# nncarlson/nka

Hardware: AMD Instinct MI355X
Metric: NKA updates/sec + achieved HBM GB/s at n=1e8, m=20 fp64; 1/2/4/8 GPUs (higher is better)
Workload: dtype f64

## Files before the change

### include/nka_hip_diag.h

```cpp
#ifndef NKA_HIP_DIAG_H
#define NKA_HIP_DIAG_H

#include "nka_hip_ext.h"
#include "nka_hip_vec.h"

#ifdef __cplusplus
extern "C" {
#endif

int nka_hip_set_tuning(nka_hip_t a, const char *key, int32_t value);

int nka_hip_get_skip_state(nka_hip_t a, int32_t out4[4]);

int nka_hip_set_grid(nka_hip_t a, int32_t pa_blocks_per_cu, int32_t pb_blocks_per_cu);

int nka_hip_debug_time_pa(nka_hip_t a, const double *f_dev, int32_t reps, float *ms_mean);

int nka_hip_debug_chain_sum(nka_hip_t a, const double *x_dev, const double *y_dev, int64_t n, double start, int32_t walk,
                            double *sum, float *ms);

int nka_hip_get_stamps(nka_hip_t a, double *out16);

int nka_hip_vec_set_tuning(nka_hip_vec_ws_t ws, const char *key, int32_t value);

#ifdef __cplusplus
}
#endif
// ... 2 lines not shown
```

### nka_amd/_lib.py

```python
from __future__ import annotations

import ctypes as C
import os
import subprocess

HERE = os.path.dirname(os.path.abspath(__file__))
_LIB = None

_i32p = C.POINTER(C.c_int32)
_dp = C.POINTER(C.c_double)
ALLREDUCE_FN = C.CFUNCTYPE(C.c_int, C.c_void_p, C.c_void_p, C.c_int32, C.c_void_p)
HOST_DOT_FN = C.CFUNCTYPE(C.c_double, C.c_void_p, C.c_int64, C.POINTER(C.c_double), C.POINTER(C.c_double))
HOST_ALLREDUCE_FN = C.CFUNCTYPE(C.c_int, C.c_void_p, C.POINTER(C.c_double), C.c_int32)

SIGNATURES = {
    "nka_hip_create": (C.c_int, [C.POINTER(C.c_void_p), C.c_int64, C.c_int32, C.c_double, C.c_int32, C.c_int32, C.c_void_p]),
    "nka_hip_destroy": (C.c_int, [C.c_void_p]),
    "nka_hip_clone": (C.c_int, [C.c_void_p, C.POINTER(C.c_void_p)]),
    "nka_hip_capture_safe": (C.c_int, [C.c_void_p]),
    "nka_hip_list_bound": (C.c_int, [C.c_void_p]),
    "nka_hip_set_stream": (C.c_int, [C.c_void_p, C.c_void_p]),
    "nka_hip_accel_update": (C.c_int, [C.c_void_p, C.c_void_p]),
    "nka_hip_accel_update_host": (C.c_int, [C.c_void_p, C.c_void_p]),
    "nka_hip_accel_update_swap": (C.c_int, [C.c_void_p, C.POINTER(C.c_void_p), C.POINTER(C.c_void_p)]),
# ... 144 lines not shown
    "nka_hip_batch_get_reductions": (C.c_int, [C.c_void_p, C.c_int32, _dp]),
    "nka_hip_batch_get_w": (C.c_int, [C.c_void_p, C.c_int32, C.c_int32, _dp]),
    "nka_hip_batch_get_v": (C.c_int, [C.c_void_p, C.c_int32, C.c_int32, _dp]),
    "nka_hip_batch_state_digest": (C.c_int, [C.c_void_p, C.c_int32, C.POINTER(C.c_uint64)]),
}


DIAG_SIGNATURES = {
    "nka_hip_set_tuning": (C.c_int, [C.c_void_p, C.c_char_p, C.c_int32]),
    "nka_hip_set_grid": (C.c_int, [C.c_void_p, C.c_int32, C.c_int32]),
    "nka_hip_debug_time_pa": (C.c_int, [C.c_void_p, C.c_void_p, C.c_int32, C.POINTER(C.c_float)]),
    "nka_hip_debug_chain_sum": (C.c_int, [C.c_void_p, C.c_void_p, C.c_void_p, C.c_int64, C.c_double, C.c_int32,
                                          C.POINTER(C.c_double), C.POINTER(C.c_float)]),
    "nka_hip_get_stamps": (C.c_int, [C.c_void_p, _dp]),
    "nka_hip_get_skip_state": (C.c_int, [C.c_void_p, C.POINTER(C.c_int32)]),
    "nka_hip_vec_set_tuning": (C.c_int, [C.c_void_p, C.c_char_p, C.c_int32]),
}
_DIAG = None


def diag_lib_path() -> str:
    return os.environ.get("NKA_HIP_DIAG_LIB") or os.path.join(HERE, "libnka_hip_diag.so")


def load_diag() -> C.CDLL:
    global _DIAG
    if _DIAG is None:
        path = diag_lib_path()
        if not os.path.exists(path):
            raise RuntimeError(f"{path} not found: `make -C nka_amd/csrc diag` (or __graft_entry__.build())")
# ... 54 lines not shown
```

### nka_amd/csrc/handles.hpp

```cpp
#pragma once

#include "../../include/nka_hip.h"
#include "../../include/nka_hip_ext.h"
#include "../../include/nka_hip_vec.h"
#include "nka_ctl.hpp"
#include "host_logic.hpp"
#include "rccl_dl.hpp"

#include <hip/hip_runtime.h>

#include <cstdint>
#include <string>
#include <vector>

namespace nka_detail {
int set_error(int code, const std::string &msg);
std::string last_error();
bool &span_check_failed();
int check_device_span(const void *p, int64_t n, const char *what);
int check_device_span_i32(const void *p, int64_t n, const char *what);
void invalidate_span_cache();
void register_allocation(const void *p, size_t bytes, const void *owner);
void unregister_owner(const void *owner);
void unregister_allocation(const void *p);
// ... 52 lines not shown
  int bpc[2] = {0, 0};
  char devname[64] = {0};
  int pa_pipe = -1;
  int pb_pipe = -1;
  int pb_flags = 0;
  int pb_tile = -1;
  int pb_tickets = -1;
  double *chain_pred = nullptr;
  void *chain_summ = nullptr;
  long long chain_cap = 0;
  int chain_many = -1;
  int chain_walk = 0;
  int fail_after_solve = 0;
  int prime_pad = -1;
  int skip_last = -1;
  int pa_skip = 0;
  bool state_in_global = false;
  bool serial_solve = false;
  int sum_order = NKA_HIP_SUMS_AUTO;
  bool debug = false;
  nka_hip_allreduce_fn allreduce = nullptr;
  void *allreduce_ctx = nullptr;
  ncclComm_t comm = nullptr;
  nka::P2P p2p{};
  void *p2p_mail = nullptr;
  std::vector<void *> p2p_opened;
  void *p2p_dev = nullptr;
  int p2p_ranks = 0;
  bool p2p_fused = false;
  int pa_normed = 0;
// ... 33 lines not shown
```

### nka_amd/csrc/lab.hip

```cpp
#include "handles.hpp"
#include "nka_chain.hpp"
#include "../../include/nka_hip_diag.h"

#include <algorithm>
#include <string>

using namespace nka;
using namespace nka_detail;

extern "C" {

int nka_hip_get_stamps(nka_hip_t a, double *out16) {
  if (!a || !out16) return fail(NKA_HIP_EINVAL, "null argument");
  HIP_TRY(hipSetDevice(a->device));
  HIP_TRY(hipMemcpyAsync(out16, a->ctl.stamps(), sizeof(double) * kStamps, hipMemcpyDeviceToHost, a->stream));
  HIP_TRY(hipStreamSynchronize(a->stream));
  return 0;
}

int nka_hip_get_skip_state(nka_hip_t a, int32_t out4[4]) {
  if (!a || !out4) return fail(NKA_HIP_EINVAL, "null argument");
  HIP_TRY(hipSetDevice(a->device));
  HIP_TRY(hipMemcpyAsync(out4, a->ctl.ic + IC_PLAN_SKIP, sizeof(int32_t) * 4, hipMemcpyDeviceToHost, a->stream));
  HIP_TRY(hipStreamSynchronize(a->stream));
  return 0;
}

int nka_hip_set_grid(nka_hip_t a, int32_t pa, int32_t pb) {
  if (!a) return fail(NKA_HIP_EINVAL, "null handle");
  const int32_t v[2] = {pa, pb};
  for (int i = 0; i < 2; i++) {
    if (v[i] < 0 || v[i] * a->num_cu > kMaxGrid) return fail(NKA_HIP_EINVAL, "blocks per CU out of range");
    a->bpc[i] = v[i];
  }
  return 0;
}

int nka_hip_debug_chain_sum(nka_hip_t a, const double *x, const double *y, int64_t n, double start, int32_t walk, double *sum,
                            float *ms) {
// ... 71 lines not shown
  } else if (k == "pb_tile") {
    if (value != -1 && value != 1 && value != 2) return fail(NKA_HIP_EINVAL, "pb_tile: -1 (auto), 1, 2");
    a->pb_tile = value;
  } else if (k == "pb_tickets") {
    if (value != -1 && value != 0 && value != 1 && value != 2 && value != 4 && value != 8)
      return fail(NKA_HIP_EINVAL, "pb_tickets: -1 (auto), 0 (static tile mapping), 1, 2, 4, 8 (ticket counters)");
    a->pb_tickets = value;
  } else if (k == "fail_after_solve") {
    a->fail_after_solve = value != 0;
  } else if (k == "prime_pad") {
    if (value < -1 || value > 1) return fail(NKA_HIP_EINVAL, "prime_pad: -1, 0, 1");
    a->prime_pad = value;
  } else if (k == "skip_last") {
    if (value < -1 || value > 1) return fail(NKA_HIP_EINVAL, "skip_last: -1, 0, 1");
    a->skip_last = value;
  } else if (k == "chain_many") {
    if (value < -1 || value > 1) return fail(NKA_HIP_EINVAL, "chain_many: -1, 0, 1");
    a->chain_many = value;
  } else if (k == "chain_walk") {
    a->chain_walk = value != 0;
  } else if (k == "serial_solve") {
    a->serial_solve = value != 0;
  } else if (k == "list_word") {
    a->word_off = value == 0;
  } else {
    return fail(NKA_HIP_EINVAL, "unknown tuning key: " + k);
  }
  return 0;
}

// ... 13 lines not shown
```

### nka_amd/csrc/nka_ctl.hpp

```cpp
#pragma once

#include <cstddef>
#include <cstdint>

#if defined(__HIPCC__)
#include <hip/hip_runtime.h>
#define NKA_HOST_DEVICE __host__ __device__
#else
#define NKA_HOST_DEVICE
#endif

namespace nka {

enum {
  IC_SUBSPACE = 0,
  IC_PENDING = 1,
  IC_FIRST = 2,
  IC_LAST = 3,
  IC_FREE = 4,
  IC_NEW = 5,
  IC_NCOMB = 6,
  IC_PLAN_PENDING = 7,
  IC_PLAN_FIRST = 8,
  IC_PLAN_NOLDER = 9,
// ... 1 lines not shown
  IC_NORMED = 11,
  IC_PLAN_SKIP = 12,
  IC_SKIP_HOLD = 13,
  IC_REDO = 14,
  IC_NREDO = 15,
  IC_HEADER = 16
};
enum { DC_VTOL = 0, DC_S = 1, DC_HEADER = 2 };
enum {
  PC_FIRST_W = 0,
  PC_NEW_W = 1,
  PC_NEW_V = 2,
  PC_OLD_W = 3,
  PC_OLD_V = 4,
  PC_WGT = 5,
  PC_HEADER = 8
};

constexpr int kMaxPerPass = 32;
constexpr int kMaxGrid = 4096;

constexpr int kStamps = 16;

struct Ctl {
  int32_t *ic;
  double *dc;
  int32_t mvec;
  unsigned long long *hw;
  unsigned long long seq;
  long long *pc;
  NKA_HOST_DEVICE long long *plan_w() const { return pc + PC_HEADER; }
  NKA_HOST_DEVICE long long *comb_w() const { return plan_w() + m1p(); }
  NKA_HOST_DEVICE long long *comb_v() const { return comb_w() + m1p(); }
  NKA_HOST_DEVICE long long *wtab() const { return comb_v() + m1p(); }
  NKA_HOST_DEVICE long long *vtab() const { return wtab() + (m1() + 1); }
  NKA_HOST_DEVICE constexpr int pc_count() const { return PC_HEADER + 3 * m1p() + 2 * (m1() + 1); }
  NKA_HOST_DEVICE constexpr int m1() const { return mvec + 1; }
  NKA_HOST_DEVICE constexpr int m1p() const { return mvec + 1 + kMaxPerPass; }
  NKA_HOST_DEVICE int32_t *next() const { return ic + IC_HEADER; }
  NKA_HOST_DEVICE int32_t *prev() const { return next() + (m1() + 1); }
  NKA_HOST_DEVICE int32_t *plan_slots() const { return prev() + (m1() + 1); }
  NKA_HOST_DEVICE int32_t *comb_slots() const { return plan_slots() + m1p(); }
  NKA_HOST_DEVICE constexpr int ic_count() const { return IC_HEADER + 2 * (m1() + 1) + 2 * m1p(); }
  NKA_HOST_DEVICE double *h() const { return dc + DC_HEADER; }
  NKA_HOST_DEVICE double *c() const { return h() + (m1() + 1) * (m1() + 1); }
  NKA_HOST_DEVICE double *comb_c() const { return c() + (m1() + 1); }
  NKA_HOST_DEVICE double *red() const { return comb_c() + m1p(); }
  NKA_HOST_DEVICE constexpr int red_count() const { return 2 + 2 * mvec; }
  NKA_HOST_DEVICE double *stamps() const { return red() + red_count(); }
  NKA_HOST_DEVICE constexpr int dc_count() const {
    return DC_HEADER + (m1() + 1) * (m1() + 1) + (m1() + 1) + m1p() + red_count() + kStamps;
// ... 24 lines not shown
```

### nka_amd/csrc/nka_hip.hip

```cpp
#include "handles.hpp"
#include "nka_kernels.hpp"

#include <dlfcn.h>

#include <algorithm>
#include <atomic>
#include <chrono>
#include <cmath>
#include <cstdio>
#include <cstdlib>
#include <cstring>
#include <map>
#include <mutex>
#include <set>
#include <string>
#include <vector>

using namespace nka;

namespace {
thread_local std::string g_err;
}

namespace nka_detail {
// ... 237 lines not shown
  if constexpr (COMB == 2) {
    if (maxk <= 4) return launch_combine_1<4, VEC, COMB>(a, f, pass, last);
    return launch_combine_1<32, VEC, COMB>(a, f, pass, last);
  }
#define CASE(K) \
  case K: return launch_combine_1<K, VEC, COMB>(a, f, pass, last);
  switch (maxk) {
    CASE(4) CASE(8) CASE(12) CASE(16) CASE(20) CASE(24) CASE(28) CASE(32)
  }
#undef CASE
  return 0;
}

template <int MAXK, int COMB, int W, int T = 1>
int launch_combine_win_1(const nka_hip_state *a, double *f, int bpc, int base) {
  static const int occ = occupancy_of(k_combine_win<MAXK, COMB, W, T>);
  const int64_t ntile = a->n / (kBlock * 2 * T);
  const int g = persistent_grid(a->num_cu, std::min(occ, std::max(1, bpc)), ntile);
  constexpr int words = ((COMB == 2 ? MAXK + 2 : 2 * MAXK + 1) + 5) * T;
  const int ng = nka_host::ticket_counters(a->pb_tickets, a->tickets != nullptr, ntile, T, g, words);
  const int tail = (ntile * (kBlock * 2 * T) < a->n) ? 1 : 0;
  hipLaunchKernelGGL((k_combine_win<MAXK, COMB, W, T>), dim3(g + tail), dim3(kBlock), 0, a->stream, a->ctl, a->vs, f,
                     ng > 0 ? a->tickets : nullptr, std::max(ng, 1), a->pb_flags, base);
  return g;
}

bool pb_tickets_apply(const nka_hip_state *a) {
  return nka_host::tickets_expected(a->pb_tickets, a->tickets != nullptr, a->n / (kBlock * 2), a->num_cu);
}

// ... 277 lines not shown
  hipFree(a->tickets);
  hipFree(a->ctl.pc);
  for (void *p : a->extra_allocs) hipFree(p);
  if (a->list_word) hipHostFree(a->list_word);
  hipFree(a->f_stage);
  hipFree(a->hd_scratch);
  hipFree(a->wgt);
  hipFree(a->wgt_chk);
  for (auto &e : a->ev)
    if (e) hipEventDestroy(e);
  a->ev.clear();
  delete a;
  return 0;
}

static int fetch_tables(nka_hip_t a, std::vector<long long> &pc, Ctl &t) {
  pc.assign((size_t)a->ctl.pc_count(), 0);
  HIP_TRY(hipMemcpyAsync(pc.data(), a->ctl.pc, sizeof(long long) * pc.size(), hipMemcpyDeviceToHost, a->stream));
  HIP_TRY(hipStreamSynchronize(a->stream));
  t = a->ctl;
  t.pc = pc.data();
  return 0;
}
static const double *slot_buffer(nka_hip_t a, const Ctl *tables, bool v, int slot) {
  if (tables) return buffer_at(a, v ? tables->vtab()[slot] : tables->wtab()[slot]);
  return (v ? a->vs.v : a->vs.w) + (size_t)(slot - 1) * a->vs.stride;
}
static __global__ void k_plan_pointers_from_slots(Ctl ctl) {
  if (threadIdx.x != 0 || blockIdx.x != 0) return;
  const int n = ctl.ic[IC_PLAN_NOLDER];
  for (int j = 0; j < n; j++) ctl.plan_w()[j] = ctl.wtab()[ctl.plan_slots()[j]];
  ctl.pc[PC_FIRST_W] = ctl.wtab()[ctl.ic[IC_PLAN_FIRST]];
}

int nka_hip_clone(nka_hip_t src, nka_hip_t *out) {
  if (!src || !out) return fail(NKA_HIP_EINVAL, "nka_hip_clone: null argument");
  *out = nullptr;
  nka_hip_t b = nullptr;
  if (int rc = nka_hip_create(&b, src->n, src->mvec, src->vtol, src->flavor, src->device, (void *)src->stream)) return rc;
  if (b->vs.stride != src->vs.stride || b->ctl.ic_count() != src->ctl.ic_count() || b->ctl.dc_count() != src->ctl.dc_count()) {
    nka_hip_destroy(b);
    return fail(NKA_HIP_ESTATE, "nka_hip_clone: storage geometry differs");
  }
  const size_t slot_bytes = (size_t)src->vs.stride * sizeof(double) * (size_t)(src->mvec + 1);
  hipStream_t s = src->stream;
  hipError_t e = hipSuccess;
  if (!src->swapped) {
    e = hipMemcpyAsync(b->vs.v, src->vs.v, slot_bytes, hipMemcpyDeviceToDevice, s);
    if (e == hipSuccess) e = hipMemcpyAsync(b->vs.w, src->vs.w, slot_bytes, hipMemcpyDeviceToDevice, s);
  } else {
    std::vector<long long> pc;
    Ctl t{};
// ... 16 lines not shown
  }
  if (e != hipSuccess) {
    nka_hip_destroy(b);
    return fail(NKA_HIP_EHIP, std::string("nka_hip_clone: ") + hipGetErrorString(e));
  }
  b->pending = src->pending;
  b->list_ub = src->list_ub;
  b->bpc[0] = src->bpc[0];
  b->bpc[1] = src->bpc[1];
  b->pa_pipe = src->pa_pipe;
  b->pb_pipe = src->pb_pipe;
  b->pb_tile = src->pb_tile;
  b->pb_tickets = src->pb_tickets;
  b->prime_pad = src->prime_pad;
  b->skip_last = src->skip_last;
  b->chain_walk = src->chain_walk;
  b->chain_many = src->chain_many;
  b->chain_pred = nullptr; b->chain_summ = nullptr; b->chain_cap = 0;
  b->serial_solve = src->serial_solve;
  b->sum_order = src->sum_order;
  b->shard_rank = src->shard_rank;
  b->shard_n = src->shard_n;
  b->debug = src->debug;
  if (src->allreduce != rccl_allreduce && src->allreduce != p2p_allreduce) {
    b->allreduce = src->allreduce;
    b->allreduce_ctx = src->allreduce_ctx;
    b->needs_comm = src->needs_comm;
  } else {
    b->needs_comm = true;
  }
// ... 8 lines not shown
    if (e != hipSuccess) {
      (void)hipGetLastError();
      nka_hip_destroy(b);
      return fail(e == hipErrorOutOfMemory ? NKA_HIP_ENOMEM : NKA_HIP_EHIP, std::string("nka_hip_clone: ") + hipGetErrorString(e));
    }
  }
  b->weighted = src->weighted;
  *out = b;
  return 0;
}

int nka_hip_restart(nka_hip_t a) {
  if (!a) return fail(NKA_HIP_EINVAL, "null handle");
  if (a->poisoned) return fail(NKA_HIP_ESTATE, "restart: an earlier update failed after its scalar step had been enqueued: destroy the handle");
  HIP_TRY(hipSetDevice(a->device));
  hipLaunchKernelGGL(k_restart, dim3(1), dim3(kSolveThreads), a->state_in_global ? 0 : lst_smem_bytes(a->mvec), a->stream,
                     a->ctl, a->state_in_global ? 1 : 0);
  HIP_TRY(hipGetLastError());
  a->pending = false;
  a->list_ub = 0;
  a->word_valid_after = a->seq;
  a->relaxed_after.clear();
  return 0;
}

int nka_hip_relax(nka_hip_t a) {
  if (!a) return fail(NKA_HIP_EINVAL, "null handle");
  if (a->poisoned) return fail(NKA_HIP_ESTATE, "relax: an earlier update failed after its scalar step had been enqueued: destroy the handle");
  HIP_TRY(hipSetDevice(a->device));
  hipLaunchKernelGGL(k_relax, dim3(1), dim3(kSolveThreads), a->state_in_global ? 0 : lst_smem_bytes(a->mvec), a->stream,
                     a->ctl, a->state_in_global ? 1 : 0);
  HIP_TRY(hipGetLastError());
  if (a->pending) {
    a->pending = false;
    a->list_ub = std::max(a->list_ub - 1, 0);
    if (!a->word_off && a->list_word) a->relaxed_after.push_back(a->seq);
    if (a->relaxed_after.size() > 4096) a->relaxed_after.erase(a->relaxed_after.begin(), a->relaxed_after.begin() + 2048);
  }
  return 0;
}

int nka_hip_set_vec_tol(nka_hip_t a, double vtol) {
  if (!a) return fail(NKA_HIP_EINVAL, "null handle");
  if (!(vtol > 0.0)) return fail(NKA_HIP_EINVAL, "set_vec_tol: vtol must be > 0");
// ... 2 lines not shown
  HIP_TRY(hipMemcpyAsync(a->ctl.dc + DC_VTOL, &a->vtol, sizeof(double), hipMemcpyHostToDevice, a->stream));
  HIP_TRY(hipStreamSynchronize(a->stream));
  return 0;
}

static int enqueue_solve(nka_hip_t a, int mode, long long swap_w = kNoBuffer, long long swap_v = kNoBuffer, bool gather = false,
                         int skip = 0) {
  hipStream_t s = a->stream;
  const P2P x = gather ? a->p2p : P2P{};
  if (a->mvec + 1 <= kSolveWaveMax && !a->serial_solve) {
    const size_t sm = solve_wave_smem_bytes(a->mvec);
    const int nl = a->mvec + 1;
    const long long id_stride = (a->swapped || a->captured) ? 0 : (long long)a->vs.stride, id_vbase = buffer_offset(a, a->vs.v);
#define ROWS(NL) \
  hipLaunchKernelGGL((k_solve_rows<NL>), dim3(1), dim3(kSolveThreads), sm, s, a->ctl, mode, swap_w, swap_v, id_stride, id_vbase, x, \
                     skip)
    if (nl <= 6) ROWS(6);
    else if (nl <= 11) ROWS(11);
    else if (nl <= 21) ROWS(21);
    else if (nl <= 33) ROWS(33);
    else if (nl <= 48) ROWS(48);
    else {
      if (!a->solve63_raised) {
        const hipError_t raised = hipFuncSetAttribute(reinterpret_cast<const void *>(k_solve_rows<63>),
                                                      hipFuncAttributeMaxDynamicSharedMemorySize,
                                                      (int)solve_wave_smem_bytes(kSolveWaveMax - 1));
        if (raised != hipSuccess) return fail(NKA_HIP_EHIP, std::string("raising the dynamic LDS limit failed: ") + hipGetErrorString(raised));
        a->solve63_raised = true;
      }
      ROWS(63);
    }
// ... 403 lines not shown
}

static int update_impl(nka_hip_t a, double *f, long long swap_w, long long swap_v);
static int p2p_status_after_sync(nka_hip_t a);

constexpr double kSkipLastMinBytes = 4.8e7;
static bool skip_last_applies(const nka_hip_state *a, SumsStage stage, int vec, int older_ub) {
  if (a->skip_last == 0) return false;
  if (stage != SumsStage::Rounded && stage != SumsStage::Blocked) return false;
  if (a->allreduce || a->host_dot || a->serial_solve) return false;
  if (a->mvec < 2 || a->mvec > kMaxPerPass || vec != 2 || older_ub != a->mvec) return false;
  if (a->pa_pipe != -1 && a->pa_pipe != 201) return false;
  return a->skip_last > 0 || 8.0 * (double)a->n >= kSkipLastMinBytes;
}

int nka_hip_accel_update(nka_hip_t a, double *f) { return update_impl(a, f, kNoBuffer, kNoBuffer); }

static int update_impl(nka_hip_t a, double *f, long long swap_w, long long swap_v) {
  if (!a) return fail(NKA_HIP_EINVAL, "null handle");
  if (!f && a->n > 0) return fail(NKA_HIP_EINVAL, "accel_update: f is NULL");
  HIP_TRY(hipSetDevice(a->device));
  if (int rc = nka_detail::check_device_span(f, a->n, "accel_update: f")) return rc;
  if (swap_w == kNoBuffer && f && f == a->last_acc)
    return fail(NKA_HIP_EINVAL, "accel_update: that buffer is the accelerated f lent by the previous out-of-place update (read only: "
                                "it is the stored v of the pending pair); copy it, or go on with nka_hip_accel_update_swap");
  if (a->poisoned)
    return fail(NKA_HIP_ESTATE, "accel_update: an earlier update of this handle failed after its scalar step had been enqueued "
                                "(a HIP error): the lists on the device are ahead of the stored vectors.  Destroy the handle");
  if (a->swapped && f && held_by_library(a, f))
    return fail(NKA_HIP_EINVAL, "accel_update: that buffer is held by the library (a stored vector, or a buffer handed over to "
// ... 19 lines not shown
    if (!a->captured || user_hook || a->host_dot) {
      hipStreamCaptureStatus cs = hipStreamCaptureStatusNone;
      if (hipStreamIsCapturing(s, &cs) != hipSuccess) (void)hipGetLastError();
      else if (cs != hipStreamCaptureStatusNone) {
        if (user_hook || a->host_dot)
          return fail(NKA_HIP_EINVAL, "accel_update: cannot be captured into a graph with a caller's all-reduce hook or dot product "
                                      "installed (host callbacks: a replay would not call them); the built-in RCCL hook and the "
                                      "peer-to-peer exchange can be captured");
        a->captured = a->word_off = true;
      }
    }
  }
  if (int rc = record(a, 0)) return rc;
  a->list_ub = list_bound_now(a);
  const int older_ub = a->pending ? std::max(a->list_ub - 1, 0) : a->list_ub;

  SumsResult sums{};
  const SumsStage stage = pick_sums_stage(a);
  const bool skip = skip_last_applies(a, stage, vec, older_ub);
  a->pa_skip = skip ? kSkipMay : 0;
  switch (stage) {
    case SumsStage::HostDot:        sums = sums_host_dot(a, f, mode); break;
    case SumsStage::ReferenceChain: sums = sums_reference_chain(a, f, mode, older_ub); break;
    case SumsStage::ReferenceOrder: sums = sums_reference_order(a, f, mode, older_ub); break;
    case SumsStage::Rounded:        sums = sums_rounded(a, f, vec, mode, older_ub); break;
    case SumsStage::Blocked:        sums = sums_blocked(a, f, vec, older_ub); break;
  }
  a->pa_skip = 0;
  if (sums.rc) return sums.rc;
  mode |= sums.mode_bits;
// ... 10 lines not shown
  } poison{a};
  if (a->fail_after_solve) {
    a->fail_after_solve = 0;
    return fail(NKA_HIP_EHIP, "accel_update: injected failure behind the scalar step (lab switch fail_after_solve)");
  }
  if (skip) {
    a->pa_skip = kSkipRepair;
    a->pa_normed = stage == SumsStage::Rounded ? ((mode & kSolveRcp) ? 3 : 1) : 0;
    launch_dots_win(1, a, f, 1, a->mvec - 1, 1, a->mvec);
    a->pa_skip = a->pa_normed = 0;
    HIP_TRY(hipGetLastError());
    if (int rc = enqueue_solve(a, mode, swap_w, swap_v, false, kSkipRepair)) return rc;
  }
  if (int rc = record(a, 2)) return rc;

  const int comb_ub = a->pending ? std::min(a->list_ub, (int)a->mvec) : a->list_ub;
  a->ctl.seq = (unsigned long long)(a->seq + 1);
  {
    Ctl &c = a->ctl;
    unsigned long long *const hw = c.hw;
    if (a->word_off) c.hw = nullptr;
    a->pb_flags = (swap_w != kNoBuffer ? (kPbNoStoreW | kPbNoStoreF) : 0);
    const int rc = enqueue_pb(a, f, vec, comb_ub);
    a->pb_flags = 0;
    c.hw = hw;
    if (rc) return rc;
  }
  a->seq++;
  if (int rc = record(a, 3)) return rc;

  if (a->timing_this) a->timing_count++;
  a->list_ub = comb_ub + 1;
  a->pending = true;
  if (swap_w == kNoBuffer) a->last_acc = nullptr;
  poison.armed = false;
  return 0;
}

int nka_hip_accel_update_host(nka_hip_t a, double *f_host) {
  if (!a) return fail(NKA_HIP_EINVAL, "null handle");
  if (!f_host && a->n > 0) return fail(NKA_HIP_EINVAL, "accel_update_host: f is NULL");
  HIP_TRY(hipSetDevice(a->device));
// ... 47 lines not shown
    }
  }
  return 0;
}

int nka_hip_accel_update_swap(nka_hip_t a, double **f_io, const double **f_acc) {
  if (!a) return fail(NKA_HIP_EINVAL, "null handle");
  if (!f_io || !f_acc || (!*f_io && a->n > 0)) return fail(NKA_HIP_EINVAL, "accel_update_swap: null argument");
  if (a->host_dot) return fail(NKA_HIP_ESTATE, "accel_update_swap: not with a user dot product on host copies (nka_hip_set_host_dot)");
  if (reinterpret_cast<uintptr_t>(*f_io) % 16 != 0) return fail(NKA_HIP_EINVAL, "accel_update_swap: the buffer must be 16-byte aligned");
  HIP_TRY(hipSetDevice(a->device));
  hipStreamCaptureStatus cs = hipStreamCaptureStatusNone;
  if (hipStreamIsCapturing(a->stream, &cs) != hipSuccess) (void)hipGetLastError();
  else if (cs != hipStreamCaptureStatusNone)
    return fail(NKA_HIP_ESTATE, "accel_update_swap: cannot be captured into a graph (the host chooses buffers per call)");
  if (int rc = collect_spares(a)) return rc;
  double *const in = *f_io, *const give_w = a->spare_w, *const vnew = a->spare_v;
  if (in && (in == give_w || in == vnew)) return fail(NKA_HIP_EINVAL, "accel_update_swap: that buffer is the library's own spare");
  if (in && in == a->last_acc)
    return fail(NKA_HIP_EINVAL, "accel_update_swap: that buffer is the accelerated f lent by the previous update (read only: it "
                                "is the stored v of the pending pair)");
  if (in && held_by_library(a, in))
    return fail(NKA_HIP_EINVAL, "accel_update_swap: that buffer is already held by the library (a stored vector, or a buffer "
                                "handed over earlier): two slots would share it");
  a->swapped = true;
  if (int rc = update_impl(a, in, buffer_offset(a, in), buffer_offset(a, vnew))) return rc;
  if (in) {
    a->book.lent.erase(in);
    const int64_t block = a->vs.stride * (int64_t)(a->mvec + 1);
    const bool inside = (in >= a->vs.w && in < a->vs.w + block) || (in >= a->vs.v && in < a->vs.v + block);
// ... 97 lines not shown
    if (last != k) return 0;
  }
  for (int k = fr; k != 0; k = next[k]) {
    if (tag[k]) return 0;
    tag[k] = 1;
  }
  for (int k = 1; k <= n; k++)
    if (!tag[k]) return 0;
  return 1;
}

static int get_slot(nka_hip_t a, bool v, int32_t slot, double *host_out) {
  if (!a) return fail(NKA_HIP_EINVAL, "null handle");
  if (slot < 1 || slot > a->mvec + 1) return fail(NKA_HIP_EINVAL, "slot out of range");
  HIP_TRY(hipSetDevice(a->device));
  std::vector<long long> pc;
  Ctl t{};
  if (a->swapped)
    if (int rc = fetch_tables(a, pc, t)) return rc;
  HIP_TRY(hipMemcpyAsync(host_out, slot_buffer(a, a->swapped ? &t : nullptr, v, slot), sizeof(double) * (size_t)a->n,
                         hipMemcpyDeviceToHost, a->stream));
  HIP_TRY(hipStreamSynchronize(a->stream));
  return 0;
}
int nka_hip_get_w(nka_hip_t a, int32_t slot, double *host_out) { return get_slot(a, false, slot, host_out); }
int nka_hip_get_v(nka_hip_t a, int32_t slot, double *host_out) { return get_slot(a, true, slot, host_out); }


int nka_hip_set_allreduce(nka_hip_t a, nka_hip_allreduce_fn fn, void *ctx) {
  if (!a) return fail(NKA_HIP_EINVAL, "null handle");
// ... 382 lines not shown
```

### nka_amd/csrc/nka_kernels.hpp

```cpp
#pragma once

#include "nka_chain.hpp"

namespace nka {


__global__ __launch_bounds__(128) void k_p2p_allreduce(P2P x, double *buf, int count) {
  const unsigned long long seq = *x.xseq;
  for (int i = threadIdx.x; i < count * x.n; i += blockDim.x) p2p_send_one(x, i % x.n, seq, i / x.n, buf[i / x.n]);
  __syncthreads();
  p2p_gather_block(x, buf, count);
}

template <int MAXL, int VEC, bool WGT = false>
__global__ __launch_bounds__(kBlock) void k_dots(Ctl ctl, Vecs vs, const double *__restrict__ f,
                                                 double *__restrict__ partials, int pass, int normed) {
  const double *wgt = WGT ? vs.w + ctl.pc[PC_WGT] : nullptr;
  using V = typename VecT<VEC>::type;
  constexpr int NACC = 2 * MAXL + 2;
  const int G = gridDim.x;
  const double s_n = normed ? sqrt(ctl.red()[0]) : 1.0, rs_n = 1.0 / s_n;
  const int pending = ctl.ic[IC_PLAN_PENDING];
  const int nolder = ctl.ic[IC_PLAN_NOLDER];
  const int base = pass * MAXL;
// ... 572 lines not shown
    chain_load_block(cs, regs, e0, lane, false);
    chain_store_block(cs, regs, blk_lds, lane);
    a = chain_block_serial(a, blk_lds, (int)(cs.n - e0));
  }
  if (lane == 0) red[cs.dst] = a;
#ifdef NKA_CHAIN_STAMPS
  if (lane == 0 && set == kChainProbe) {
    for (int i = 0; i < 8; i++) ctl.stamps()[8 + i] = (double)cnt[i];
    ctl.stamps()[3] = (double)tw;
  }
#endif
#undef NKA_APPLY_COUNT
}

enum { kPbNoStoreW = 1, kPbNoStoreF = 2,
       kPbNotFirst = 8, kPbNotLast = 16 };

template <int MAXK, int VEC, int COMB>
__global__ __launch_bounds__(kBlock) void k_combine(Ctl ctl, Vecs vs, double *f, int pass, int last_pass, int flags) {
  using V = typename VecT<VEC>::type;
  constexpr bool RCP = (COMB == 1);
  constexpr bool COMPACT = (COMB == 2);
  constexpr int NW = COMPACT ? 1 : MAXK;
  const int G = gridDim.x;
  const int ncomb = ctl.ic[IC_NCOMB];
  double *wnew = vs.w + ctl.pc[PC_NEW_W], *vnew = vs.w + ctl.pc[PC_NEW_V];
  const long long *cw = ctl.comb_w(), *cv = ctl.comb_v();
  const double *cc = ctl.comb_c();
  const int base = pass * MAXK;
  const bool oop = (flags & kPbNoStoreF) != 0;
  const double *src = (oop && pass > 0) ? vnew : f;
// ... 68 lines not shown
            v = RCP ? rs * v : v / s;
            if (COMPACT) v = v - w;
            wk[0][i] = w;
            vk[0][i] = v;
          }
          x = COMPACT ? x + ck[j] * v : comb1<COMB>(x, ck[j], w, v);
        }
      }
      if (store_w) wnew[i] = fin;
      if (store_v) vnew[i] = x;
      if (store_f) f[i] = x;
    }
  }
}

template <int MAXK, int COMB, int W, int T = 1>
__global__ __launch_bounds__(kBlock) void k_combine_win(Ctl ctl, Vecs vs, double *f, unsigned *tickets, int ng, int flags,
                                                        int base) {
  constexpr int VEC = 2;
  using V = typename VecT<VEC>::type;
  constexpr bool RCP = (COMB == 1);
  constexpr bool COMPACT = (COMB == 2);
  constexpr int TILE = kBlock * VEC * T;
  static_assert(MAXK % W == 0, "the ring must divide the pairs of a tile");
  NKA_STAMP0(ctl, 14);
  __shared__ unsigned s_next[2];
  const int64_t ntile = vs.n / TILE;
  const bool has_tail = ntile * TILE < vs.n;
  const int G = (int)gridDim.x - (has_tail ? 1 : 0);
  const bool tail_block = has_tail && (int)blockIdx.x == G;
  const int ncomb_all = ctl.ic[IC_NCOMB];
  const int ncomb = ncomb_all - base;
  double *wnew = vs.w + ctl.pc[PC_NEW_W], *vnew = vs.w + ctl.pc[PC_NEW_V];
  const long long *cw = ctl.comb_w() + base, *cv = ctl.comb_v() + base;
  const double *cc = ctl.comb_c() + base;
  const bool first_pass = !(flags & kPbNotFirst), last_pass = !(flags & kPbNotLast);
  const bool store_w = !(flags & kPbNoStoreW) && first_pass, store_f = !(flags & kPbNoStoreF), store_v = last_pass;
  const bool norm0 = first_pass && ctl.ic[IC_NORMED] != 0;
  const double s = ctl.dc[DC_S];
  const double rs = 1.0 / s;

  double *wk[MAXK], *vk[MAXK];
  double ck[MAXK];
  long long slw[MAXK], slv[MAXK];
#pragma unroll
  for (int j = 0; j < MAXK; j++) {
    if (!COMPACT || j == 0) slw[j] = cw[j];
    slv[j] = cv[j];
    ck[j] = cc[j];
  }
#pragma unroll
  for (int j = 0; j < MAXK; j++) {
    const bool live = j < ncomb;
// ... 210 lines not shown

constexpr int kSolveWaveMax = 63;

__host__ __device__ inline size_t solve_wave_smem_bytes(int mvec) {
  const int nl = mvec + 1;
  size_t b = (lst_smem_bytes(mvec) + 15) / 16 * 16;
  b += (size_t)((nl + 1) * (nl + 1) + 3 * nl + (2 + 2 * mvec)) * sizeof(double);
  b += (size_t)(3 * nl + 1) * sizeof(int32_t);
  b = (b + 7) / 8 * 8;
  b += (size_t)(2 * (nl + 1)) * sizeof(long long);
  return b;
}

template <int NLMAX>
__global__ __launch_bounds__(kSolveThreads) void k_solve_rows(Ctl ctl, int mode, long long swap_w, long long swap_v,
                                                              long long id_stride, long long id_vbase, P2P x, int skip) {
  extern __shared__ __attribute__((aligned(16))) unsigned char smem[];
  const int lane = threadIdx.x;
  if (skip_repair_idle(ctl, skip)) return;
  if (x.base != nullptr) p2p_gather_block(x, ctl.red(), ctl.red_count());
  const int m1 = ctl.m1(), NL = m1, LDA = NL + 1, M = ctl.mvec, nh = (m1 + 1) * (m1 + 1);
  Lst L;
  L.m1 = m1;
  L.mvec = M;
  L.h = reinterpret_cast<double *>(smem);
  L.c = L.h + nh;
  L.next = reinterpret_cast<int32_t *>(L.c + (m1 + 1));
  L.prev = L.next + (m1 + 1);
  double *A = reinterpret_cast<double *>(smem + (lst_smem_bytes(ctl.mvec) + 15) / 16 * 16);
  double *bb = A + (NL + 1) * LDA + 2 * NL;
  double *redL = bb + NL;
  int32_t *ord = reinterpret_cast<int32_t *>(redL + (2 + 2 * M));
  int32_t *psL = ord + 2 * NL;
  long long *wtL = reinterpret_cast<long long *>((reinterpret_cast<uintptr_t>(psL + NL + 1) + 7) / 8 * 8);
// ... 201 lines not shown
      }
    }
    NKA_STAMP(ctl, 7);
    nk = __builtin_popcountll(alive & listmask);
    if (lane < nl && ((alive >> lane) & 1)) {
      const int r = __builtin_popcountll(alive & ((1ull << lane) - 1));
      ctl.comb_slots()[r] = myord;
      ctl.comb_c()[r] = yr;
      ctl.plan_slots()[r] = myord;
      const long long wb = wtL[myord];
      ctl.comb_w()[r] = wb;
      ctl.comb_v()[r] = vtL[myord];
      ctl.plan_w()[r] = wb;
      L.c[myord] = yr;
    }
  } else if (L.subspace) {
    for (int k = L.first; k != 0; k = L.next[k]) ord[nk++] = k;
    __syncthreads();
    for (int p = lane; p < nk; p += kSolveThreads) bb[p] = L.c[ord[p]];
    for (int idx = lane; idx < nk * nk; idx += kSolveThreads) {
      const int p = idx / nk, q = idx - p * nk;
      if (p >= q) A[p * LDA + q] = L.H(ord[p], ord[q]);
    }
    __syncthreads();
    for (int i = 0; i < nk; i++) {
      const double ci = bb[i] / A[i * LDA + i];
      __syncthreads();
      if (lane == 0) bb[i] = ci;
      for (int j = i + 1 + lane; j < nk; j += kSolveThreads) bb[j] = bb[j] - A[j * LDA + i] * ci;
      __syncthreads();
// ... 25 lines not shown
    if (entry_first != 0 && !normed && entry_pending) ctl.ic[IC_NRELAX] += 1;
    ctl.ic[IC_NEW] = slot;
    ctl.ic[IC_NCOMB] = nk;
    ctl.ic[IC_NORMED] = normed;
    lst_store_scalars(L, ctl);
    ctl.ic[IC_PLAN_PENDING] = L.pending;
    ctl.ic[IC_PLAN_FIRST] = L.first;
    ctl.ic[IC_PLAN_NOLDER] = nk;
    int hold = hold_in > 0 ? hold_in - 1 : 0;
    if (skip & kSkipRepair) {
      hold = M;
      ctl.ic[IC_REDO] = 0;
    }
    ctl.ic[IC_SKIP_HOLD] = hold;
    ctl.ic[IC_PLAN_SKIP] = hold == 0 ? 1 : 0;
  }
  NKA_STAMP(ctl, 9);
}

}
```

### nka_amd/nka.py

```python
from __future__ import annotations

import ctypes as C

import numpy as np

from . import _lib

FLAVOR_F08, FLAVOR_F08_VECTOR, FLAVOR_C = 0, 1, 2
FLAVOR_DEFAULT = -1
SUMS_AUTO, SUMS_REFERENCE_ORDER, SUMS_BLOCKED, SUMS_BLOCKED_ROUNDED = 0, 1, 2, 3


class NKAError(RuntimeError):
    pass


def _check(rc: int, what: str, L=None):
    if rc != 0:
        msg = (L or _lib.load()).nka_hip_last_error()
        raise NKAError(f"{what} failed ({rc}): {msg.decode() if msg else ''}")


class State:

# ... 356 lines not shown

    def set_grid(self, pa=0, pb=0):
        self._need_diag("set_grid")
        _check(self._L.nka_hip_set_grid(self._handle(), pa, pb), "set_grid", self._L)

    def set_tuning(self, key: str, value: int):
        self._need_diag("set_tuning")
        _check(self._L.nka_hip_set_tuning(self._handle(), key.encode(), int(value)), "set_tuning", self._L)

    def skip_state(self):
        self._need_diag("skip_state")
        out = (C.c_int32 * 4)()
        _check(self._L.nka_hip_get_skip_state(self._handle(), out), "get_skip_state", self._L)
        return tuple(out)

    def debug_chain_sum(self, x, y, start: float = 0.0, walk: bool = False, many: bool = False):
        self._need_diag("debug_chain_sum")
        assert x.dtype == y.dtype and x.numel() == y.numel() and x.is_contiguous() and y.is_contiguous()
        out, ms = C.c_double(), C.c_float()
        _check(self._L.nka_hip_debug_chain_sum(self._handle(), x.data_ptr(), y.data_ptr(), x.numel(), float(start),
                                               int(bool(walk)) | (2 if many else 0), C.byref(out), C.byref(ms)), "debug_chain_sum", self._L)
        return out.value, ms.value

    def device_info(self):
        name = C.create_string_buffer(64)
        ncu = C.c_int32()
        _check(self._L.nka_hip_device_info(self._handle(), name, C.byref(ncu)), "device_info", self._L)
        return name.value.decode(), ncu.value
```

Measured before the change: 134.8.

## Defer materialising the new v vector and replay it in the next combine pass

Adds a deferred-v mode for the C flavor with compact storage. The combine kernel skips storing the new v vector, and the next update's combine recomputes its contribution on the fly from the saved previous coefficients, or a materialise kernel builds it when v is needed elsewhere. This removes one full n-length store per update, and possibly a later reload, at the cost of more arithmetic, extra reads of the kept vectors, extra control-table state and more complex correctness paths. It is gated on default heuristics such as vector size and ticket use.

```diff
diff --git a/include/nka_hip_diag.h b/include/nka_hip_diag.h
--- a/include/nka_hip_diag.h
+++ b/include/nka_hip_diag.h
@@ -11,6 +11,8 @@
 int nka_hip_set_tuning(nka_hip_t a, const char *key, int32_t value);
 
 int nka_hip_get_skip_state(nka_hip_t a, int32_t out4[4]);
+
+int nka_hip_get_defer_state(nka_hip_t a, int32_t out2[2]);
 
 int nka_hip_set_grid(nka_hip_t a, int32_t pa_blocks_per_cu, int32_t pb_blocks_per_cu);
 
diff --git a/nka_amd/_lib.py b/nka_amd/_lib.py
--- a/nka_amd/_lib.py
+++ b/nka_amd/_lib.py
@@ -182,6 +182,7 @@
                                           C.POINTER(C.c_double), C.POINTER(C.c_float)]),
     "nka_hip_get_stamps": (C.c_int, [C.c_void_p, _dp]),
     "nka_hip_get_skip_state": (C.c_int, [C.c_void_p, C.POINTER(C.c_int32)]),
+    "nka_hip_get_defer_state": (C.c_int, [C.c_void_p, C.POINTER(C.c_int32)]),
     "nka_hip_vec_set_tuning": (C.c_int, [C.c_void_p, C.c_char_p, C.c_int32]),
 }
 _DIAG = None
diff --git a/nka_amd/csrc/handles.hpp b/nka_amd/csrc/handles.hpp
--- a/nka_amd/csrc/handles.hpp
+++ b/nka_amd/csrc/handles.hpp
@@ -90,6 +90,9 @@
   int fail_after_solve = 0;
   int prime_pad = -1;
   int skip_last = -1;
+  int defer_v = -1;
+  bool v_deferred = false;
+  bool pb_defer = false;
   int pa_skip = 0;
   bool state_in_global = false;
   bool serial_solve = false;
diff --git a/nka_amd/csrc/lab.hip b/nka_amd/csrc/lab.hip
--- a/nka_amd/csrc/lab.hip
+++ b/nka_amd/csrc/lab.hip
@@ -23,6 +23,17 @@
   HIP_TRY(hipSetDevice(a->device));
   HIP_TRY(hipMemcpyAsync(out4, a->ctl.ic + IC_PLAN_SKIP, sizeof(int32_t) * 4, hipMemcpyDeviceToHost, a->stream));
   HIP_TRY(hipStreamSynchronize(a->stream));
+  return 0;
+}
+
+int nka_hip_get_defer_state(nka_hip_t a, int32_t out2[2]) {
+  if (!a || !out2) return fail(NKA_HIP_EINVAL, "null argument");
+  HIP_TRY(hipSetDevice(a->device));
+  long long w[2] = {0, 0};
+  HIP_TRY(hipMemcpyAsync(w, a->ctl.pc + PC_VDEFER, sizeof w, hipMemcpyDeviceToHost, a->stream));
+  HIP_TRY(hipStreamSynchronize(a->stream));
+  out2[0] = (int32_t)w[0];
+  out2[1] = (int32_t)w[1];
   return 0;
 }
 
@@ -124,6 +135,9 @@
   } else if (k == "skip_last") {
     if (value < -1 || value > 1) return fail(NKA_HIP_EINVAL, "skip_last: -1, 0, 1");
     a->skip_last = value;
+  } else if (k == "defer_v") {
+    if (value < -1 || value > 1) return fail(NKA_HIP_EINVAL, "defer_v: -1, 0, 1");
+    a->defer_v = value;
   } else if (k == "chain_many") {
     if (value < -1 || value > 1) return fail(NKA_HIP_EINVAL, "chain_many: -1, 0, 1");
     a->chain_many = value;
diff --git a/nka_amd/csrc/nka_ctl.hpp b/nka_amd/csrc/nka_ctl.hpp
--- a/nka_amd/csrc/nka_ctl.hpp
+++ b/nka_amd/csrc/nka_ctl.hpp
@@ -39,6 +39,8 @@
   PC_OLD_W = 3,
   PC_OLD_V = 4,
   PC_WGT = 5,
+  PC_VDEFER = 6,
+  PC_VREPLAY = 7,
   PC_HEADER = 8
 };
 
@@ -59,7 +61,11 @@
   NKA_HOST_DEVICE long long *comb_v() const { return comb_w() + m1p(); }
   NKA_HOST_DEVICE long long *wtab() const { return comb_v() + m1p(); }
   NKA_HOST_DEVICE long long *vtab() const { return wtab() + (m1() + 1); }
-  NKA_HOST_DEVICE constexpr int pc_count() const { return PC_HEADER + 3 * m1p() + 2 * (m1() + 1); }
+  NKA_HOST_DEVICE long long *rp_v() const { return vtab() + (m1() + 1); }
+  NKA_HOST_DEVICE double *rp_cprev() const { return reinterpret_cast<double *>(rp_v() + m1p()); }
+  NKA_HOST_DEVICE double *rp_cnew() const { return rp_cprev() + m1p(); }
+  NKA_HOST_DEVICE long long *rp_keep() const { return rp_v() + 3 * m1p(); }
+  NKA_HOST_DEVICE constexpr int pc_count() const { return PC_HEADER + 3 * m1p() + 2 * (m1() + 1) + 3 * m1p() + 1; }
   NKA_HOST_DEVICE constexpr int m1() const { return mvec + 1; }
   NKA_HOST_DEVICE constexpr int m1p() const { return mvec + 1 + kMaxPerPass; }
   NKA_HOST_DEVICE int32_t *next() const { return ic + IC_HEADER; }
diff --git a/nka_amd/csrc/nka_hip.hip b/nka_amd/csrc/nka_hip.hip
--- a/nka_amd/csrc/nka_hip.hip
+++ b/nka_amd/csrc/nka_hip.hip
@@ -275,6 +275,18 @@
 
 template <int MAXK, int COMB, int W, int T = 1>
 int launch_combine_win_1(const nka_hip_state *a, double *f, int bpc, int base) {
+  if constexpr (COMB == 2) {
+    if (a->pb_defer) {
+      static const int occ_d = occupancy_of(k_combine_win<MAXK, COMB, W, T, true>);
+      const int64_t ntile = a->n / (kBlock * 2 * T);
+      const int g = persistent_grid(a->num_cu, std::min(occ_d, std::max(1, bpc)), ntile);
+      const int ng = nka_host::ticket_counters(a->pb_tickets, a->tickets != nullptr, ntile, T, g, (MAXK + 2 + 5) * T);
+      const int tail = (ntile * (kBlock * 2 * T) < a->n) ? 1 : 0;
+      hipLaunchKernelGGL((k_combine_win<MAXK, COMB, W, T, true>), dim3(g + tail), dim3(kBlock), 0, a->stream, a->ctl, a->vs, f,
+                         ng > 0 ? a->tickets : nullptr, std::max(ng, 1), a->pb_flags | kPbMayDefer, base);
+      return g;
+    }
+  }
   static const int occ = occupancy_of(k_combine_win<MAXK, COMB, W, T>);
   const int64_t ntile = a->n / (kBlock * 2 * T);
   const int g = persistent_grid(a->num_cu, std::min(occ, std::max(1, bpc)), ntile);
@@ -582,6 +594,8 @@
   return 0;
 }
 
+static int ensure_v(nka_hip_t a, bool clear_only = false);
+
 static int fetch_tables(nka_hip_t a, std::vector<long long> &pc, Ctl &t) {
   pc.assign((size_t)a->ctl.pc_count(), 0);
   HIP_TRY(hipMemcpyAsync(pc.data(), a->ctl.pc, sizeof(long long) * pc.size(), hipMemcpyDeviceToHost, a->stream));
@@ -604,6 +618,8 @@
 int nka_hip_clone(nka_hip_t src, nka_hip_t *out) {
   if (!src || !out) return fail(NKA_HIP_EINVAL, "nka_hip_clone: null argument");
   *out = nullptr;
+  HIP_TRY(hipSetDevice(src->device));
+  if (int rc = ensure_v(src)) return rc;
   nka_hip_t b = nullptr;
   if (int rc = nka_hip_create(&b, src->n, src->mvec, src->vtol, src->flavor, src->device, (void *)src->stream)) return rc;
   if (b->vs.stride != src->vs.stride || b->ctl.ic_count() != src->ctl.ic_count() || b->ctl.dc_count() != src->ctl.dc_count()) {
@@ -650,6 +666,7 @@
   b->pb_tickets = src->pb_tickets;
   b->prime_pad = src->prime_pad;
   b->skip_last = src->skip_last;
+  b->defer_v = src->defer_v;
   b->chain_walk = src->chain_walk;
   b->chain_many = src->chain_many;
   b->chain_pred = nullptr; b->chain_summ = nullptr; b->chain_cap = 0;
@@ -688,6 +705,7 @@
   if (!a) return fail(NKA_HIP_EINVAL, "null handle");
   if (a->poisoned) return fail(NKA_HIP_ESTATE, "restart: an earlier update failed after its scalar step had been enqueued: destroy the handle");
   HIP_TRY(hipSetDevice(a->device));
+  if (int rc = ensure_v(a, true)) return rc;
   hipLaunchKernelGGL(k_restart, dim3(1), dim3(kSolveThreads), a->state_in_global ? 0 : lst_smem_bytes(a->mvec), a->stream,
                      a->ctl, a->state_in_global ? 1 : 0);
   HIP_TRY(hipGetLastError());
@@ -702,6 +720,7 @@
   if (!a) return fail(NKA_HIP_EINVAL, "null handle");
   if (a->poisoned) return fail(NKA_HIP_ESTATE, "relax: an earlier update failed after its scalar step had been enqueued: destroy the handle");
   HIP_TRY(hipSetDevice(a->device));
+  if (int rc = ensure_v(a, true)) return rc;
   hipLaunchKernelGGL(k_relax, dim3(1), dim3(kSolveThreads), a->state_in_global ? 0 : lst_smem_bytes(a->mvec), a->stream,
                      a->ctl, a->state_in_global ? 1 : 0);
   HIP_TRY(hipGetLastError());
@@ -734,7 +753,7 @@
     const long long id_stride = (a->swapped || a->captured) ? 0 : (long long)a->vs.stride, id_vbase = buffer_offset(a, a->vs.v);
 #define ROWS(NL) \
   hipLaunchKernelGGL((k_solve_rows<NL>), dim3(1), dim3(kSolveThreads), sm, s, a->ctl, mode, swap_w, swap_v, id_stride, id_vbase, x, \
-                     skip)
+                     skip, a->pb_defer ? 1 : 0)
     if (nl <= 6) ROWS(6);
     else if (nl <= 11) ROWS(11);
     else if (nl <= 21) ROWS(21);
@@ -1168,6 +1187,31 @@
   return a->skip_last > 0 || 8.0 * (double)a->n >= kSkipLastMinBytes;
 }
 
+constexpr double kDeferVMinBytes = 1.6e7;
+static bool defer_v_applies(const nka_hip_state *a, int vec, long long swap_w, int comb_ub) {
+  if (a->defer_v == 0) return false;
+  if (a->flavor != NKA_HIP_FLAVOR_C || swap_w != kNoBuffer || vec != 2) return false;
+  if (a->mvec > kMaxPerPass || comb_ub > kMaxPerPass) return false;
+  if (a->captured || a->host_dot || a->serial_solve) return false;
+  if (a->pb_pipe != -1 && !(a->pb_pipe > 200 && a->pb_pipe < 210)) return false;
+  if (a->pb_tickets == 0 || !a->tickets) return false;
+  if (a->defer_v > 0) return true;
+  return pb_tickets_apply(a) && 8.0 * (double)a->n >= kDeferVMinBytes;
+}
+
+static int ensure_v(nka_hip_t a, bool clear_only) {
+  if (!a->v_deferred) return 0;
+  const int64_t nb = (a->n + kBlock - 1) / kBlock;
+  const int g = (int)std::max<int64_t>(1, std::min<int64_t>(nb, (int64_t)a->num_cu * 8));
+  if (!clear_only) hipLaunchKernelGGL(k_materialise_v, dim3(g), dim3(kBlock), 0, a->stream, a->ctl, a->vs, 0);
+  hipLaunchKernelGGL(k_materialise_v, dim3(1), dim3(64), 0, a->stream, a->ctl, a->vs, 1);
+  HIP_TRY(hipGetLastError());
+  hipStreamCaptureStatus cs = hipStreamCaptureStatusNone;
+  if (hipStreamIsCapturing(a->stream, &cs) != hipSuccess) (void)hipGetLastError();
+  else if (cs == hipStreamCaptureStatusNone) a->v_deferred = false;
+  return 0;
+}
+
 int nka_hip_accel_update(nka_hip_t a, double *f) { return update_impl(a, f, kNoBuffer, kNoBuffer); }
 
 static int update_impl(nka_hip_t a, double *f, long long swap_w, long long swap_v) {
@@ -1217,6 +1261,15 @@
   if (int rc = record(a, 0)) return rc;
   a->list_ub = list_bound_now(a);
   const int older_ub = a->pending ? std::max(a->list_ub - 1, 0) : a->list_ub;
+  const int comb_ub = a->pending ? std::min(a->list_ub, (int)a->mvec) : a->list_ub;
+  const bool defer = defer_v_applies(a, vec, swap_w, comb_ub);
+  if (!defer)
+    if (int rc = ensure_v(a)) return rc;
+  struct DeferScope {
+    nka_hip_state *a;
+    ~DeferScope() { a->pb_defer = false; }
+  } defer_scope{a};
+  a->pb_defer = defer;
 
   SumsResult sums{};
   const SumsStage stage = pick_sums_stage(a);
@@ -1257,7 +1310,6 @@
   }
   if (int rc = record(a, 2)) return rc;
 
-  const int comb_ub = a->pending ? std::min(a->list_ub, (int)a->mvec) : a->list_ub;
   a->ctl.seq = (unsigned long long)(a->seq + 1);
   {
     Ctl &c = a->ctl;
@@ -1269,6 +1321,7 @@
     c.hw = hw;
     if (rc) return rc;
   }
+  if (defer) a->v_deferred = true;
   a->seq++;
   if (int rc = record(a, 3)) return rc;
 
@@ -1346,6 +1399,7 @@
   if (hipStreamIsCapturing(a->stream, &cs) != hipSuccess) (void)hipGetLastError();
   else if (cs != hipStreamCaptureStatusNone)
     return fail(NKA_HIP_ESTATE, "accel_update_swap: cannot be captured into a graph (the host chooses buffers per call)");
+  if (int rc = ensure_v(a)) return rc;
   if (int rc = collect_spares(a)) return rc;
   double *const in = *f_io, *const give_w = a->spare_w, *const vnew = a->spare_v;
   if (in && (in == give_w || in == vnew)) return fail(NKA_HIP_EINVAL, "accel_update_swap: that buffer is the library's own spare");
@@ -1473,6 +1527,13 @@
   if (!a) return fail(NKA_HIP_EINVAL, "null handle");
   if (slot < 1 || slot > a->mvec + 1) return fail(NKA_HIP_EINVAL, "slot out of range");
   HIP_TRY(hipSetDevice(a->device));
+  if (v && a->v_deferred) {
+    int32_t first = 0;
+    HIP_TRY(hipMemcpyAsync(&first, a->ctl.ic + IC_FIRST, sizeof first, hipMemcpyDeviceToHost, a->stream));
+    HIP_TRY(hipStreamSynchronize(a->stream));
+    if (slot == first)
+      if (int rc = ensure_v(a)) return rc;
+  }
   std::vector<long long> pc;
   Ctl t{};
   if (a->swapped)
diff --git a/nka_amd/csrc/nka_kernels.hpp b/nka_amd/csrc/nka_kernels.hpp
--- a/nka_amd/csrc/nka_kernels.hpp
+++ b/nka_amd/csrc/nka_kernels.hpp
@@ -610,7 +610,8 @@
 }
 
 enum { kPbNoStoreW = 1, kPbNoStoreF = 2,
-       kPbNotFirst = 8, kPbNotLast = 16 };
+       kPbNotFirst = 8, kPbNotLast = 16,
+       kPbMayDefer = 32 };
 
 template <int MAXK, int VEC, int COMB>
 __global__ __launch_bounds__(kBlock) void k_combine(Ctl ctl, Vecs vs, double *f, int pass, int last_pass, int flags) {
@@ -709,7 +710,186 @@
   }
 }
 
-template <int MAXK, int COMB, int W, int T = 1>
+template <int MAXK, int W, int T>
+__device__ __forceinline__ void combine_win_replay(const Ctl &ctl, const Vecs &vs, double *f, unsigned *tickets, int ng, int flags,
+                                                   int np, unsigned *s_next) {
+  constexpr int VEC = 2;
+  using V = typename VecT<VEC>::type;
+  constexpr int TILE = kBlock * VEC * T;
+  const int64_t ntile = vs.n / TILE;
+  const bool has_tail = ntile * TILE < vs.n;
+  const int G = (int)gridDim.x - (has_tail ? 1 : 0);
+  const bool tail_block = has_tail && (int)blockIdx.x == G;
+  const int ncomb = ctl.ic[IC_NCOMB];
+  double *wnew = vs.w + ctl.pc[PC_NEW_W], *vnew = vs.w + ctl.pc[PC_NEW_V];
+  double *w1 = vs.w + ctl.comb_w()[0], *u1 = vs.w + ctl.comb_v()[0];
+  const double c0 = ctl.comb_c()[0];
+  const unsigned keep = (unsigned)ctl.rp_keep()[0];
+  const bool store_w = !(flags & kPbNoStoreW), store_f = !(flags & kPbNoStoreF);
+  const bool store_v = !((flags & kPbMayDefer) && ncomb > 0);
+  const double s = ctl.dc[DC_S];
+  __shared__ double s_cf[2 * MAXK];
+  for (int j = threadIdx.x; j < 2 * MAXK; j += kBlock) {
+    const int k = j < MAXK ? j : j - MAXK;
+    s_cf[j] = k < np ? (j < MAXK ? ctl.rp_cprev()[k] : ctl.rp_cnew()[k]) : 0.0;
+  }
+  __syncthreads();
+  double cp[MAXK], cn[MAXK];
+  const double *uk[MAXK];
+  long long slv[MAXK];
+#pragma unroll
+  for (int j = 0; j < MAXK; j++) {
+    cp[j] = s_cf[j];
+    cn[j] = s_cf[MAXK + j];
+    slv[j] = ctl.rp_v()[j];
+  }
+#pragma unroll
+  for (int j = 0; j < MAXK; j++) uk[j] = j < np ? vs.w + slv[j] : f;
+
+  const int lane_off = threadIdx.x * VEC;
+#define DEAD_OFF(live, off) ((live) ? (off) : (int64_t)lane_off)
+  V finv[T], w0v[T], rv[W][T];
+  int64_t t = tail_block ? ntile : (int64_t)blockIdx.x;
+  if (t < ntile) {
+    const int64_t e = t * TILE + lane_off;
+#pragma unroll
+    for (int q = 0; q < T; q++) {
+      finv[q] = ld<VEC>(f + e + q * (kBlock * VEC));
+      w0v[q] = ld<VEC>(w1 + e + q * (kBlock * VEC));
+    }
+#pragma unroll
+    for (int j = 0; j < W; j++)
+#pragma unroll
+      for (int q = 0; q < T; q++) rv[j][q] = ld<VEC>(uk[j] + DEAD_OFF(j < np, e) + q * (kBlock * VEC));
+  }
+  list_word_publish(ctl, ncomb, flags & kPbNoStoreW);
+  const unsigned grp = tickets ? blockIdx.x % (unsigned)ng : 0u;
+  unsigned *const my_ticket = tickets ? tickets + grp * kTicketStride : nullptr;
+  const unsigned ticket_base = tickets ? 2u * (unsigned)G / (unsigned)ng : 0u;
+  int64_t tnext = t + G;
+  unsigned par = 0;
+  while (t < ntile) {
+    const int64_t e = t * TILE + lane_off;
+    const bool more = tnext < ntile;
+    unsigned claimed = kNoTicket;
+    if (tickets && more && threadIdx.x == 0) claimed = ticket_request(my_ticket, ticket_base, (unsigned)ng, grp);
+    const int64_t tn = more ? tnext : t;
+    const int64_t en = tn * TILE + lane_off;
+    V fin[T], w0[T], v1[T], x[T], kept[MAXK][T];
+#pragma unroll
+    for (int q = 0; q < T; q++) {
+      fin[q] = finv[q];
+      w0[q] = w0v[q];
+      v1[q] = w0[q];
+      if (store_w) st(wnew + e + q * (kBlock * VEC), fin[q]);
+    }
+    __builtin_amdgcn_sched_barrier(0);
+#pragma unroll
+    for (int q = 0; q < T; q++) {
+      finv[q] = ld<VEC>(f + en + q * (kBlock * VEC));
+      w0v[q] = ld<VEC>(w1 + en + q * (kBlock * VEC));
+    }
+#pragma unroll
+    for (int j = 0; j < MAXK; j++) {
+#pragma unroll
+      for (int q = 0; q < T; q++) kept[j][q] = rv[j % W][q];
+      __builtin_amdgcn_sched_barrier(0);
+#pragma unroll
+      for (int q = 0; q < T; q++) {
+        if (j + W < MAXK) rv[j % W][q] = ld<VEC>(uk[j + W] + DEAD_OFF(j + W < np, e) + q * (kBlock * VEC));
+        else rv[j % W][q] = ld<VEC>(uk[j + W - MAXK] + DEAD_OFF(j + W - MAXK < np, en) + q * (kBlock * VEC));
+      }
+      __builtin_amdgcn_sched_barrier(0);
+      if (j < np) {
+#pragma unroll
+        for (int q = 0; q < T; q++)
+#pragma unroll
+          for (int c = 0; c < VEC; c++) setc(v1[q], c, ex(v1[q], c) + cp[j] * ex(kept[j][q], c));
+      }
+    }
+#pragma unroll
+    for (int q = 0; q < T; q++) {
+      V wn, un;
+#pragma unroll
+      for (int c = 0; c < VEC; c++) {
+        const double d = ex(w0[q], c) - ex(fin[q], c);
+        const double wq = d / s;
+        const double vq = ex(v1[q], c) / s;
+        setc(wn, c, wq);
+        setc(un, c, vq - wq);
+        setc(x[q], c, ex(fin[q], c) + c0 * (vq - wq));
+      }
+      st(w1 + e + q * (kBlock * VEC), wn);
+      st(u1 + e + q * (kBlock * VEC), un);
+    }
+#pragma unroll
+    for (int j = 0; j < MAXK; j++) {
+      if (j < np && ((keep >> j) & 1u)) {
+#pragma unroll
+        for (int q = 0; q < T; q++)
+#pragma unroll
+          for (int c = 0; c < VEC; c++) setc(x[q], c, ex(x[q], c) + cn[j] * ex(kept[j][q], c));
+      }
+    }
+#pragma unroll
+    for (int q = 0; q < T; q++) {
+      if (store_v) st(vnew + e + q * (kBlock * VEC), x[q]);
+      if (store_f) st(f + e + q * (kBlock * VEC), x[q]);
+    }
+    const int64_t t2 = tickets ? ticket_publish(s_next, par, claimed, ntile) : tnext + G;
+    t = tnext;
+    tnext = t2;
+  }
+  if (tickets && !tail_block) ticket_finish(tickets, ng, G);
+  if (tail_block) {
+    for (int64_t i = ntile * TILE + threadIdx.x; i < vs.n; i += kBlock) {
+      const double fin = f[i], w0 = w1[i];
+      double v1 = w0, kept[MAXK];
+#pragma unroll
+      for (int j = 0; j < MAXK; j++) {
+        kept[j] = 0.0;
+        if (j < np) {
+          kept[j] = uk[j][i];
+          v1 = v1 + cp[j] * kept[j];
+        }
+      }
+      const double d = w0 - fin;
+      const double wq = d / s;
+      const double vq = v1 / s;
+      const double un = vq - wq;
+      w1[i] = wq;
+      u1[i] = un;
+      double x = fin + c0 * un;
+#pragma unroll
+      for (int j = 0; j < MAXK; j++)
+        if (j < np && ((keep >> j) & 1u)) x = x + cn[j] * kept[j];
+      if (store_w) wnew[i] = fin;
+      if (store_v) vnew[i] = x;
+      if (store_f) f[i] = x;
+    }
+  }
+#undef DEAD_OFF
+}
+
+__global__ __launch_bounds__(kBlock) void k_materialise_v(Ctl ctl, Vecs vs, int clear) {
+  if (ctl.pc[PC_VDEFER] == 0) return;
+  if (clear) {
+    if (blockIdx.x == 0 && threadIdx.x == 0) ctl.pc[PC_VDEFER] = 0;
+    return;
+  }
+  const int ncomb = ctl.ic[IC_NCOMB];
+  const double *w = vs.w + ctl.pc[PC_NEW_W];
+  double *v = vs.w + ctl.pc[PC_NEW_V];
+  const long long *cv = ctl.comb_v();
+  const double *cc = ctl.comb_c();
+  for (int64_t i = (int64_t)blockIdx.x * kBlock + threadIdx.x; i < vs.n; i += (int64_t)gridDim.x * kBlock) {
+    double x = w[i];
+    for (int j = 0; j < ncomb; j++) x = x + cc[j] * (vs.w + cv[j])[i];
+    v[i] = x;
+  }
+}
+
+template <int MAXK, int COMB, int W, int T = 1, bool DEFER = false>
 __global__ __launch_bounds__(kBlock) void k_combine_win(Ctl ctl, Vecs vs, double *f, unsigned *tickets, int ng, int flags,
                                                         int base) {
   constexpr int VEC = 2;
@@ -730,8 +910,18 @@
   const long long *cw = ctl.comb_w() + base, *cv = ctl.comb_v() + base;
   const double *cc = ctl.comb_c() + base;
   const bool first_pass = !(flags & kPbNotFirst), last_pass = !(flags & kPbNotLast);
-  const bool store_w = !(flags & kPbNoStoreW) && first_pass, store_f = !(flags & kPbNoStoreF), store_v = last_pass;
+  const bool store_w = !(flags & kPbNoStoreW) && first_pass, store_f = !(flags & kPbNoStoreF);
+  const bool store_v = last_pass && !(DEFER && (flags & kPbMayDefer) && ncomb_all > 0);
   const bool norm0 = first_pass && ctl.ic[IC_NORMED] != 0;
+  if constexpr (DEFER) {
+    static_assert(COMPACT, "the deferred v exists for compact storage only");
+    if (blockIdx.x == 0 && threadIdx.x == 0) ctl.pc[PC_VDEFER] = store_v ? 0 : 1;
+    const int np = norm0 ? (int)ctl.pc[PC_VREPLAY] : 0;
+    if (np > 0) {
+      combine_win_replay<MAXK, W, T>(ctl, vs, f, tickets, ng, flags, np, s_next);
+      return;
+    }
+  }
   const double s = ctl.dc[DC_S];
   const double rs = 1.0 / s;
 
@@ -972,10 +1162,17 @@
 
 template <int NLMAX>
 __global__ __launch_bounds__(kSolveThreads) void k_solve_rows(Ctl ctl, int mode, long long swap_w, long long swap_v,
-                                                              long long id_stride, long long id_vbase, P2P x, int skip) {
+                                                              long long id_stride, long long id_vbase, P2P x, int skip, int vd) {
   extern __shared__ __attribute__((aligned(16))) unsigned char smem[];
   const int lane = threadIdx.x;
   if (skip_repair_idle(ctl, skip)) return;
+  const bool vd_in = vd != 0 && ctl.pc[PC_VDEFER] != 0;
+  double vd_cprev = 0.0;
+  long long vd_v = 0;
+  if (vd != 0 && lane >= 1 && lane <= ctl.mvec) {
+    vd_cprev = ctl.comb_c()[lane - 1];
+    vd_v = ctl.comb_v()[lane - 1];
+  }
   if (x.base != nullptr) p2p_gather_block(x, ctl.red(), ctl.red_count());
   const int m1 = ctl.m1(), NL = m1, LDA = NL + 1, M = ctl.mvec, nh = (m1 + 1) * (m1 + 1);
   Lst L;
@@ -1207,6 +1404,11 @@
       ctl.plan_w()[r] = wb;
       L.c[myord] = yr;
     }
+    if (vd_in && lane >= 1 && lane < nl) {
+      ctl.rp_v()[lane - 1] = vd_v;
+      ctl.rp_cprev()[lane - 1] = vd_cprev;
+      ctl.rp_cnew()[lane - 1] = yr;
+    }
   } else if (L.subspace) {
     for (int k = L.first; k != 0; k = L.next[k]) ord[nk++] = k;
     __syncthreads();
@@ -1262,6 +1464,11 @@
     }
     ctl.ic[IC_SKIP_HOLD] = hold;
     ctl.ic[IC_PLAN_SKIP] = hold == 0 ? 1 : 0;
+    if (vd != 0) {
+      ctl.pc[PC_VREPLAY] = (vd_in && normed) ? nl - 1 : 0;
+      ctl.rp_keep()[0] = (long long)((alive & listmask) >> 1);
+      ctl.pc[PC_VDEFER] = 0;
+    }
   }
   NKA_STAMP(ctl, 9);
 }
diff --git a/nka_amd/nka.py b/nka_amd/nka.py
--- a/nka_amd/nka.py
+++ b/nka_amd/nka.py
@@ -394,6 +394,12 @@
         _check(self._L.nka_hip_get_skip_state(self._handle(), out), "get_skip_state", self._L)
         return tuple(out)
 
+    def defer_state(self):
+        self._need_diag("defer_state")
+        out = (C.c_int32 * 2)()
+        _check(self._L.nka_hip_get_defer_state(self._handle(), out), "get_defer_state", self._L)
+        return tuple(out)
+
     def debug_chain_sum(self, x, y, start: float = 0.0, walk: bool = False, many: bool = False):
         self._need_diag("debug_chain_sum")
         assert x.dtype == y.dtype and x.numel() == y.numel() and x.is_contiguous() and y.is_contiguous()
```

After: 137.0, median of 6. 1.6% higher.
